# ginevracoal/robustBNNs

Measured on AMD Instinct MI355X. Metric: attack-samples/sec (test_pts x posterior_samples x PGD_iters), higher is better.
Workload: dtype f32 (full-width operands as three f16 pieces: 6 exact f16 MFMA product terms per fp32 product, f32 accumulate)

## Files before the change

### robustbnns_amd/csrc/rbnn_triple.hip

```cpp
#include "rbnn_common.hpp"
#include <algorithm>
#include <cstdlib>

namespace {

__device__ __forceinline__ void split3(float v, _Float16& p0, _Float16& p1, _Float16& p2) {
    p0 = (_Float16)v;
    float r = v - (float)p0;
    p1 = (_Float16)r;
    r -= (float)p1;
    p2 = (_Float16)r;
}

#ifndef RBNN_X3_PAIR_NOP
#define RBNN_X3_PAIR_NOP 0
#endif
#if RBNN_X3_PAIR_NOP
#define RBNN_X3_PAIR_PAD "\n\ts_nop 1"
#else
#define RBNN_X3_PAIR_PAD ""
#endif
#define RBNN_X3_PAIR_BODY \
    "v_bfe_i32 %[me], %[mw], %[b0], 1\n\t" \
    "v_bfe_i32 %[mo], %[mw], %[b1], 1\n\t" \
// ... 27 lines not shown
    "v_fma_mix_f32 %[re], %[ge], %[me], -%[d0] op_sel_hi:[0,0,1]\n\t" \
    "v_fma_mix_f32 %[ro], %[go], %[mo], -%[d0] op_sel:[0,0,1] op_sel_hi:[0,0,1]\n\t" \
    "v_cvt_pk_f16_f32 %[d1], %[re], %[ro]\n\t" \
    "v_fma_mixlo_f16 %[d2], -%[d1], %[one], %[re] op_sel_hi:[1,0,0]\n\t" \
    "v_fma_mixhi_f16 %[d2], -%[d1], %[one], %[ro] op_sel:[1,0,0] op_sel_hi:[1,0,0]" RBNN_X3_PAIR_PAD
#define RBNN_X3_PAIRM_OPS \
    : [d0] "=&v"(d0), [d1] "=&v"(d1), [d2] "=&v"(d2), [re] "=&v"(re), [ro] "=&v"(ro) \
    : [ge] "v"(ge), [go] "v"(go), [me] "v"(me), [mo] "v"(mo), [one] "v"(one)
    if constexpr (FIRST) asm volatile("s_nop 7\n\t" RBNN_X3_PAIRM_BODY RBNN_X3_PAIRM_OPS);
    else asm volatile(RBNN_X3_PAIRM_BODY RBNN_X3_PAIRM_OPS);
}


__global__ void triple_rows_kernel(const float* __restrict__ src, long long rows, int cols, int ld_src, float scale,
                                   const rbnn_dev_scale* __restrict__ ds, uint4* __restrict__ dst, int groups, int grouped) {
    const long long i = (long long)blockIdx.x * blockDim.x + threadIdx.x;
    if (i >= rows * groups) return;
    if (ds) scale = ds->scale;
    const long long r = i / groups;
    const int g = (int)(i % groups);
    const float* const p = src + r * ld_src + 8 * g;
    union { f16x8 v; uint4 u; } o[3];
#pragma unroll
    for (int j = 0; j < 8; ++j) {
        const float v = (8 * g + j < cols) ? p[j] * scale : 0.f;
        _Float16 a, b, c;
        split3(v, a, b, c);
        o[0].v[j] = a; o[1].v[j] = b; o[2].v[j] = c;
    }
    if (grouped) {
        uint4* const out = dst + (((r >> 4) * (groups >> 2) + (g >> 2)) * 192 + (r & 15) * 4 + (g & 3));
        out[0] = o[0].u; out[64] = o[1].u; out[128] = o[2].u;
        return;
    }
    uint4* const out = dst + (r * (groups >> 2) + (g >> 2)) * 12 + (g & 3);
    out[0] = o[0].u; out[4] = o[1].u; out[8] = o[2].u;
}

struct FwdX3Args {
    const char* X;  int ldx;  int N;
    const char* W;  long long w_sample_bytes;  int ldw;  int KT;
    const float* b;  const float* W2;  const float* b2;  int C;  int H;
    const int* sidx;  int S;  int NT;  float out_scale;
    float* P;  uint32_t* mask;  float* dact;  int out_kind;
    const rbnn_dev_scale* x_ds;
    long long x_sample_bytes;  char* hid;  float hid_scale;  const rbnn_dev_scale* hid_ds;
    unsigned x_group_bytes, x_stage_bytes;
};

template <int ACT, int WH, int HTW, int WN, int NTW, bool LAYER2, bool XF32 = false>
__global__ void __launch_bounds__(64 * WH * WN, WH * WN / 4) fc_forward_x3_kernel(const FwdX3Args a) {
    constexpr int BH = WH * HTW * 16, BN = WN * NTW * 16;
    constexpr int PLANEB = (BH + BN) * 64;
    constexpr int TILEB = 3 * PLANEB;
    constexpr bool BITMASK = (ACT == RBNN_ACT_RELU || ACT == RBNN_ACT_LEAKY);
    constexpr int NW = WH * WN;
    constexpr int WPP = BH / 16 / NW, XPP = BN / 16 / NW;
    static_assert((BH / 16) % NW == 0 && (BN / 16) % NW == 0, "whole pieces per wave");
    static_assert(HTW % 2 == 0 && HTW <= 8, "a wave's h range is whole 32-bit mask words, at most 4");
    static_assert(WH * BN * 64 <= 2 * TILEB, "the Z^T reduction scratch aliases the tile buffers");
    extern __shared__ __attribute__((aligned(16))) float lds[];
    char* const ldsb = (char*)lds;
    float* const zred = lds;

    int id;
    if (!item_of_block(blockIdx.x, a.NT * a.S, id)) return;
    constexpr int SB = 4;
    int ntile, s;
    {
        const int full = a.S / SB, per = SB * a.NT;
        if (id < full * per) { ntile = (id % per) / SB; s = (id / per) * SB + id % SB; }
        else { const int rem = id - full * per, cnt = a.S - full * SB; ntile = rem / cnt; s = full * SB + rem % cnt; }
    }
    const int tid = threadIdx.x, lane = tid & 63, li = lane & 15, lg = lane >> 4;
    const int wave = __builtin_amdgcn_readfirstlane(tid >> 6);
    const int wave_h = wave % WH, wave_n = wave / WH;
    const int sw = a.sidx ? a.sidx[s] : s;
    const float out_scale = a.x_ds ? a.out_scale * a.x_ds->inv_scale : a.out_scale;
    const float hid_scale = (!LAYER2 && a.hid_ds) ? a.hid_ds->scale : a.hid_scale;
    const char* const Ws = a.W + (long long)sw * a.w_sample_bytes;
    const char* const Xs = a.X + (long long)s * a.x_sample_bytes;
    const int n0 = ntile * BN;
    const int HW = a.H >> 5;
    const int prow = lane >> 2;
    const unsigned src_off = (unsigned)(prow * 64 + ((lane & 3) ^ swz(prow)) * 16);
    const int foff = li * 64 + ((lg ^ swz(li)) * 16);
    auto sw8 = [](int r) { return ((r >> 1) & 1) | (((r >> 2) & 1) << 2); };
    const unsigned src_off_f = (unsigned)((lane >> 3) * 128 + (((lane & 7) ^ sw8(lane >> 3)) * 16));
    const int foff_f0 = li * 128 + (((2 * lg) ^ sw8(li)) * 16), foff_f1 = li * 128 + (((2 * lg + 1) ^ sw8(li)) * 16);

    f32x4 zacc[NTW];
#pragma unroll
    for (int nt = 0; nt < NTW; ++nt) zacc[nt] = (f32x4){0.f, 0.f, 0.f, 0.f};
    if (NW == 8 && wave >= 4) __builtin_amdgcn_s_setprio(1);

    unsigned xrow[XPP], wrow[WPP];
#pragma unroll
    for (int i = 0; i < XPP; ++i) xrow[i] = (unsigned)min((n0 >> 4) + wave + NW * i, ((a.N + 15) >> 4) - 1) * a.x_group_bytes + (XF32 ? src_off_f : src_off);
#pragma unroll
    for (int i = 0; i < WPP; ++i) wrow[i] = (unsigned)(wave + NW * i) * (unsigned)a.KT * 3072u + src_off;

    constexpr int PPS = WPP + XPP;
    const int G = (a.H / BH) * a.KT;
    auto piece = [&](int c, int kt, int buf, int j) {
        char* const T = ldsb + buf * TILEB;
        const char* src;
        char* dst;
        if (j < WPP) {
            src = Ws + (long long)c * BH * a.ldw * 6 + (wrow[j < WPP ? j : 0] + (unsigned)kt * 3072u);
            dst = T + (wave + NW * j) * 3072;
        } else {
            src = Xs + (xrow[j >= WPP ? j - WPP : 0] + (unsigned)kt * a.x_stage_bytes);
            dst = T + (BH / 16 + wave + NW * (j - WPP)) * 3072;
        }
        const auto gsrc = (const __attribute__((address_space(1))) void*)src;
        const auto ldst = (__attribute__((address_space(3))) void*)(uintptr_t)(uint32_t)(uintptr_t)dst;
        __builtin_amdgcn_global_load_lds(gsrc, ldst, 16, 0, 0);
        __builtin_amdgcn_global_load_lds(gsrc, ldst, 16, 1024, 0);
        if (!(XF32 && j >= WPP)) __builtin_amdgcn_global_load_lds(gsrc, ldst, 16, 2048, 0);
    };
#pragma unroll
    for (int i = 0; i < PPS; ++i) piece(0, 0, 0, i);
    ring_wait_barrier<0>();

    f32x4 acc[HTW][NTW];
#pragma unroll
    for (int ht = 0; ht < HTW; ++ht)
#pragma unroll
        for (int nt = 0; nt < NTW; ++nt) acc[ht][nt] = (f32x4){0.f, 0.f, 0.f, 0.f};

    int kt = 0, ch = 0;
    for (int g = 0; g < G; ++g) {
        const int buf = g & 1;
        const bool wrap = kt + 1 == a.KT, last = g + 1 == G;
        const int ktn = last ? kt : (wrap ? 0 : kt + 1), chn = (wrap && !last) ? ch + 1 : ch;
        const char* const Wt = ldsb + buf * TILEB + (wave_h * HTW) * 3072 + foff;
        const char* const Xt = ldsb + buf * TILEB + (BH / 16 + wave_n * NTW) * 3072 + foff;
        f16x8 b0[NTW], b1[NTW], b2[NTW], a0, a1, a2, a0n, a1n, a2n;
        if (!(RBNN_ABL & 1)) {
#pragma unroll
            for (int i = 0; i < PPS; ++i) piece(chn, ktn, buf ^ 1, i);
        }
        if constexpr (XF32) {
            const char* const Xf = ldsb + buf * TILEB + (BH / 16 + wave_n * NTW) * 3072;
            f32x4 x0[NTW], x1[NTW];
#pragma unroll
            for (int nt = 0; nt < NTW; ++nt) {
                x0[nt] = *(const f32x4*)(Xf + nt * 3072 + foff_f0);
                x1[nt] = *(const f32x4*)(Xf + nt * 3072 + foff_f1);
            }
#pragma unroll
            for (int nt = 0; nt < NTW; ++nt) {
                union { f16x8 v; unsigned w[4]; } q0, q1, q2;
                split3_plain_pair(x0[nt][0], x0[nt][1], 1.f, q0.w[0], q1.w[0], q2.w[0]);
                split3_plain_pair(x0[nt][2], x0[nt][3], 1.f, q0.w[1], q1.w[1], q2.w[1]);
                split3_plain_pair(x1[nt][0], x1[nt][1], 1.f, q0.w[2], q1.w[2], q2.w[2]);
                split3_plain_pair(x1[nt][2], x1[nt][3], 1.f, q0.w[3], q1.w[3], q2.w[3]);
                b0[nt] = q0.v; b1[nt] = q1.v; b2[nt] = q2.v;
            }
        } else {
#pragma unroll
            for (int nt = 0; nt < NTW; ++nt) {
                b0[nt] = *(const f16x8*)(Xt + nt * 3072);
                b1[nt] = *(const f16x8*)(Xt + nt * 3072 + 1024);
                b2[nt] = *(const f16x8*)(Xt + nt * 3072 + 2048);
            }
        }
        a0 = *(const f16x8*)(Wt);
        a1 = *(const f16x8*)(Wt + 1024);
        a2 = *(const f16x8*)(Wt + 2048);
        a0n = a0; a1n = a1; a2n = a2;
#pragma unroll
        for (int ht = 0; ht < HTW; ++ht) {
#pragma unroll
            for (int k = 0; k < 6; ++k) {
                const f16x8 av = (k == 1) ? a2 : ((k == 2 || k == 3) ? a1 : a0);
#pragma unroll
                for (int nt = 0; nt < NTW; ++nt) {
                    const f16x8 bv = (k == 0) ? b2[nt] : ((k == 2 || k == 4) ? b1[nt] : b0[nt]);
                    acc[ht][nt] = MFMA_H(av, bv, acc[ht][nt]);
                }
                if (k == 0 && ht + 1 < HTW) {
                    a0n = *(const f16x8*)(Wt + (ht + 1) * 3072);
                    a1n = *(const f16x8*)(Wt + (ht + 1) * 3072 + 1024);
                    a2n = *(const f16x8*)(Wt + (ht + 1) * 3072 + 2048);
                }
            }
            a0 = a0n; a1 = a1n; a2 = a2n;
        }
        {
            __builtin_amdgcn_sched_group_barrier(0x100, 3 * NTW + 3, 0);
#pragma unroll
            for (int ht = 0; ht < HTW; ++ht) {
                __builtin_amdgcn_sched_group_barrier(0x008, 3 * NTW, 0);
                if (ht + 1 < HTW) __builtin_amdgcn_sched_group_barrier(0x100, 3, 0);
                __builtin_amdgcn_sched_group_barrier(0x008, 3 * NTW, 0);
            }
        }
        if (!(RBNN_ABL & 2)) ring_wait_barrier<0>();
        const int hc0 = ch * BH;
        kt = wrap ? 0 : kt + 1;
        ch = wrap ? ch + 1 : ch;
        if (!wrap) continue;

        if (RBNN_ABL & 8) {
            float t = 0.f;
#pragma unroll
            for (int ht = 0; ht < HTW; ++ht)
#pragma unroll
                for (int nt = 0; nt < NTW; ++nt) { t += acc[ht][nt][0] + acc[ht][nt][1] + acc[ht][nt][2] + acc[ht][nt][3]; acc[ht][nt] = (f32x4){0.f, 0.f, 0.f, 0.f}; }
            if (t == 12345.678f) a.P[tid] = t;
            continue;
        }
        const int hw0 = hc0 + (wave_h * HTW) * 16;
        unsigned mine[NTW];
#pragma unroll
        for (int nt = 0; nt < NTW; ++nt) mine[nt] = 0u;
#pragma unroll
        for (int ht = 0; ht < HTW; ++ht) {
            const int hrow = hw0 + ht * 16 + 4 * lg;
            const f32x4 bias = *(const f32x4*)(a.b + (long long)sw * a.H + hrow);
            f32x4 w2f = (f32x4){0.f, 0.f, 0.f, 0.f};
            if (LAYER2 && li < a.C) w2f = *(const f32x4*)(a.W2 + ((long long)sw * a.C + li) * a.H + hrow);
#pragma unroll
            for (int nt = 0; nt < NTW; ++nt) {
                const int n = n0 + (wave_n * NTW + nt) * 16 + li;
                f32x4 v = acc[ht][nt] * out_scale + bias, hv;
                acc[ht][nt] = (f32x4){0.f, 0.f, 0.f, 0.f};
                unsigned bits = 0;
#pragma unroll
                for (int r = 0; r < 4; ++r) {
                    bits |= (v[r] > 0.f ? 1u : 0u) << r;
                    hv[r] = act_fwd<ACT>(v[r]);
                }
                if (BITMASK) {
                    unsigned part = bits << (16 * (ht & 1) + 4 * lg);
                    part |= __shfl_xor(part, 16);
                    part |= __shfl_xor(part, 32);
                    if (lg == (ht >> 1)) mine[nt] |= part;
                }
                if (!BITMASK && a.dact && n < a.N) {
                    f32x4 dv;
#pragma unroll
                    for (int r = 0; r < 4; ++r) dv[r] = act_grad_from_value<ACT>(hv[r]);
                    *(f32x4*)(a.dact + ((long long)s * a.N + n) * a.H + hrow) = dv;
                }
                if (LAYER2) {
#pragma unroll
                    for (int r = 0; r < 4; ++r) zacc[nt] = MFMA16(w2f[r], hv[r], zacc[nt]);
                } else {
#ifdef RBNN_X3_L1_ABL_NOSTORE
                    if (n < a.N && hv[0] == 1.2345e-30f) {
#else
                    if (n < a.N) {
#endif
                        const long long blk = ((long long)s * HW + (hrow >> 5)) * ((a.N + 15) >> 4) + (n >> 4);
#ifdef RBNN_X3_L1_ABL_SMALL
                        char* const row = a.hid + ((blk * 2048) & 0xFFC00) + (n & 15) * 128 + ((hrow >> 4) & 1) * 64 + lg * 16;
#else
                        char* const row = a.hid + blk * 2048 + (n & 15) * 128 + ((hrow >> 4) & 1) * 64 + lg * 16;
#endif
                        *(f32x4*)row = hv * hid_scale;
                    }
                }
            }
        }
        if (BITMASK && a.mask) {
#pragma unroll
            for (int nt = 0; nt < NTW; ++nt) {
                const int n = n0 + (wave_n * NTW + nt) * 16 + li;
                if (lg < HTW / 2 && n < a.N) a.mask[((long long)s * HW + (hw0 >> 5) + lg) * mask_ld(a.N) + n] = mine[nt];
            }
        }
    }
    if (RBNN_ABL & 2) ring_wait_barrier<0>();

    if (!LAYER2) return;
#pragma unroll
    for (int nt = 0; nt < NTW; ++nt)
        *(f32x4*)(zred + (wave_h * BN + (wave_n * NTW + nt) * 16 + li) * 16 + 4 * lg) = zacc[nt];
    __syncthreads();
    if (tid < BN) {
        const int n = n0 + tid;
        float z[16];
#pragma unroll
        for (int q = 0; q < 4; ++q) {
            f32x4 sum = *(const f32x4*)(zred + tid * 16 + 4 * q);
#pragma unroll
            for (int w = 1; w < WH; ++w) sum += *(const f32x4*)(zred + (w * BN + tid) * 16 + 4 * q);
#pragma unroll
            for (int r = 0; r < 4; ++r) z[4 * q + r] = sum[r];
        }
        float m = -INFINITY;
#pragma unroll
        for (int c = 0; c < 16; ++c) {
            if (c < a.C) { z[c] += a.b2[(long long)sw * a.C + c]; m = fmaxf(m, z[c]); }
            else z[c] = 0.f;
        }
        if (a.out_kind == RBNN_OUT_PROBS) {
            float den = 0.f;
#pragma unroll
            for (int c = 0; c < 16; ++c) if (c < a.C) { z[c] = expf(z[c] - m); den += z[c]; }
#pragma unroll
            for (int c = 0; c < 16; ++c) if (c < a.C) z[c] = z[c] / den;
        }
        if (n < a.N) {
            float* const dst = a.P + ((long long)s * a.N + n) * RBNN_CPAD;
#pragma unroll
            for (int q = 0; q < 4; ++q) *(f32x4*)(dst + 4 * q) = (f32x4){z[4 * q], z[4 * q + 1], z[4 * q + 2], z[4 * q + 3]};
        }
    }
}

template <int ACT, int WH, int HTW, int WN, int NTW, bool LAYER2, bool XF32>
int launch_forward_x3_cfg(FwdX3Args a, hipStream_t st) {
    constexpr int BH = WH * HTW * 16, BN = WN * NTW * 16;
    constexpr int LDSB = 2 * 3 * (BH + BN) * 64;
    static_assert(LDSB <= 160 * 1024, "LDS");
    a.NT = (a.N + BN - 1) / BN;
    auto kern = fc_forward_x3_kernel<ACT, WH, HTW, WN, NTW, LAYER2, XF32>;
    static unsigned long long attr_done = 0;
    if (!ensure_dynamic_lds((const void*)kern, LDSB, attr_done)) return RBNN_ERR_LAUNCH;
    const int grid = grid_for_items((long long)a.NT * a.S);
    hipLaunchKernelGGL(kern, dim3(grid), dim3(64 * WH * WN), LDSB, st, a);
    return launch_status();
}

template <int ACT, bool LAYER2, bool XF32>
int launch_forward_x3_act(const FwdX3Args& a, hipStream_t st) {
    if (a.H % 256 == 0) return launch_forward_x3_cfg<ACT, 4, 4, 2, 4, LAYER2, XF32>(a, st);
    if (a.H % 128 == 0) return launch_forward_x3_cfg<ACT, 2, 4, 2, 4, LAYER2, XF32>(a, st);
    return RBNN_ERR_UNSUPPORTED;
}

template <bool LAYER2, bool XF32 = false>
int launch_forward_x3(int act, const FwdX3Args& a, hipStream_t st) {
    switch (act) {
#ifndef RBNN_FAST_BUILD
        case RBNN_ACT_RELU:  return launch_forward_x3_act<RBNN_ACT_RELU, LAYER2, XF32>(a, st);
#endif
        case RBNN_ACT_LEAKY: return launch_forward_x3_act<RBNN_ACT_LEAKY, LAYER2, XF32>(a, st);
#ifndef RBNN_FAST_BUILD
        case RBNN_ACT_SIGM:  return launch_forward_x3_act<RBNN_ACT_SIGM, LAYER2, XF32>(a, st);
        case RBNN_ACT_TANH:  return launch_forward_x3_act<RBNN_ACT_TANH, LAYER2, XF32>(a, st);
#endif
    }
    return RBNN_ERR_UNSUPPORTED;
}

__global__ void triple_cols_kernel(const float* __restrict__ W, long long n_mats, int rows, int cols, int ld_src, float scale,
                                   uint4* __restrict__ dst, int ld_dst) {
    const long long i = (long long)blockIdx.x * blockDim.x + threadIdx.x;
    const int HB = rows / 32;
    if (i >= n_mats * HB * 4 * ld_dst) return;
    const int d = (int)(i % ld_dst);
    const int lg = (int)((i / ld_dst) % 4);
    const long long mh = i / (4LL * ld_dst);
// ... 21 lines not shown
    const int t = (int)((i >> 7) % (H / 16));
    const long long m = (i >> 7) / (H / 16);
    _Float16 w[3][10];
#pragma unroll
    for (int c = 0; c < 10; ++c) {
        const float v = (c < C) ? W2[(m * C + c) * H + 16 * t + li] * scale : 0.f;
        split3(v, w[0][c], w[1][c], w[2][c]);
    }
    union { f16x8 v; uint4 u; } o;
    const _Float16 z = (_Float16)0.f;
    if (lg < 3) {
        const int piece = (k == 0) ? (lg == 2 ? 1 : 0) : (lg == 0 ? 1 : (lg == 1 ? 0 : 2));
#pragma unroll
        for (int j = 0; j < 8; ++j) o.v[j] = piece == 0 ? w[0][j] : (piece == 1 ? w[1][j] : w[2][j]);
    } else if (k == 0) {
        o.v[0] = w[0][8]; o.v[1] = w[0][9]; o.v[2] = w[0][8]; o.v[3] = w[0][9];
        o.v[4] = w[0][8]; o.v[5] = w[0][9]; o.v[6] = w[1][8]; o.v[7] = w[1][9];
    } else {
        o.v[0] = w[2][8]; o.v[1] = w[2][9]; o.v[2] = w[1][8]; o.v[3] = w[1][9];
        o.v[4] = z; o.v[5] = z; o.v[6] = z; o.v[7] = z;
    }
    dst[i] = o.u;
}

__host__ __device__ __forceinline__ int dz_swz3(long long n) { return (int)((0 - (n >> 2)) & 3); }

__global__ void __launch_bounds__(256) triple_dz_kernel(const float* __restrict__ dZ, int S, int N, long long N_pad, int C,
                                                        uint4* __restrict__ dst, float* __restrict__ gscale) {
    __shared__ float red[16][17];
    const int p = threadIdx.x & 15, q = threadIdx.x >> 4;
    const long long n = (long long)blockIdx.x * 16 + p;
    float m = 0.f;
    if (n < N)
        for (int s = q; s < S; s += 16) {
            const float* const src = dZ + ((long long)s * N + n) * RBNN_CPAD;
#pragma unroll
            for (int k = 0; k < 3; ++k) {
                const f32x4 v = *(const f32x4*)(src + 4 * k);
#pragma unroll
                for (int r = 0; r < 4; ++r) if (4 * k + r < C) m = fmaxf(m, fabsf(v[r]));
            }
        }
    red[q][p] = m;
    __syncthreads();
    m = 0.f;
#pragma unroll
    for (int i = 0; i < 16; ++i) m = fmaxf(m, red[i][p]);
    int e = 0;
    if (m > 0.f && m < INFINITY) e = min(13 - ilogbf(m), 120);
    if (q == 0) gscale[n] = ldexpf(1.f, -e);
    const int sw = dz_swz3(n);
    for (int s = q; s < S; s += 16) {
        _Float16 d[3][10];
        float v[12];
        if (n < N) {
            const float* const src = dZ + ((long long)s * N + n) * RBNN_CPAD;
#pragma unroll
            for (int k = 0; k < 3; ++k) {
                const f32x4 t = *(const f32x4*)(src + 4 * k);
#pragma unroll
                for (int r = 0; r < 4; ++r) v[4 * k + r] = t[r];
            }
        }
#pragma unroll
        for (int c = 0; c < 10; ++c) {
            const float x = (n < N && c < C) ? ldexpf(v[c], e) : 0.f;
            split3(x, d[0][c], d[1][c], d[2][c]);
        }
        uint4* const o = dst + ((long long)s * N_pad + n) * 4;
#pragma unroll
        for (int ch = 0; ch < 3; ++ch) {
            union { f16x8 v; uint4 u; } w;
#pragma unroll
            for (int j = 0; j < 8; ++j) w.v[j] = d[ch][j];
            o[ch ^ sw] = w.u;
        }
        union { f16x8 v; uint4 u; } t;
        t.v[0] = d[0][8]; t.v[1] = d[0][9]; t.v[2] = d[1][8]; t.v[3] = d[1][9];
        t.v[4] = d[2][8]; t.v[5] = d[2][9]; t.v[6] = d[0][8]; t.v[7] = d[0][9];
        o[3 ^ sw] = t.u;
    }
}

template <int MODE>
__device__ __forceinline__ void tail_dz(const float* __restrict__ prow, const float (&gmean)[16], int y, int C, float inv_S, float (&out)[16]) {
    float p[16], g[16];
#pragma unroll
    for (int q = 0; q < 4; ++q) {
        const f32x4 v = *(const f32x4*)(prow + 4 * q);
#pragma unroll
        for (int r = 0; r < 4; ++r) p[4 * q + r] = v[r];
    }
    if (MODE == RBNN_LOSS_PER_SAMPLE) {
        ce_softmax_grad<16>(p, C, y, inv_S, g);
    } else {
#pragma unroll
        for (int c = 0; c < 16; ++c) g[c] = gmean[c];
    }
    if (MODE == RBNN_LOSS_MEAN_LOGIT) {
#pragma unroll
        for (int c = 0; c < 16; ++c) out[c] = g[c];
    } else {
        softmax_backward<16>(g, p, C, out);
    }
}

template <int MODE>
__global__ void __launch_bounds__(256) step_tail_x3_kernel(const float* __restrict__ P, const int* __restrict__ labels, int S, float inv_S, int N,
                                                           long long N_pad, int C, float* __restrict__ Psum_out, int ldo,
                                                           uint4* __restrict__ dst, float* __restrict__ gscale) {
    __shared__ float red[16][17];
    __shared__ float psum[16][16];
    const int p = threadIdx.x & 15, q = threadIdx.x >> 4;
    const long long n = (long long)blockIdx.x * 16 + p;
    if (MODE != RBNN_LOSS_PER_SAMPLE) {
        if (q < 4) {
            f32x4 sum = (f32x4){0.f, 0.f, 0.f, 0.f};
            if (n < N)
                for (int s = 0; s < S; ++s) sum += *(const f32x4*)(P + ((long long)s * N + n) * RBNN_CPAD + 4 * q);
#pragma unroll
            for (int r = 0; r < 4; ++r) {
                psum[p][4 * q + r] = sum[r];
                if (Psum_out && n < N && 4 * q + r < C) Psum_out[n * ldo + 4 * q + r] = sum[r];
            }
        }
        __syncthreads();
    }
    const int y = (n < N) ? labels[n] : 0;
    float gmean[16];
    if (MODE != RBNN_LOSS_PER_SAMPLE) {
        float t[16];
#pragma unroll
        for (int c = 0; c < 16; ++c) t[c] = (c < C) ? psum[p][c] * inv_S : 0.f;
        ce_softmax_grad<16>(t, C, y, inv_S, gmean);
    } else {
#pragma unroll
        for (int c = 0; c < 16; ++c) gmean[c] = 0.f;
    }
    float m = 0.f;
    if (n < N)
        for (int s = q; s < S; s += 16) {
            float dz[16];
            tail_dz<MODE>(P + ((long long)s * N + n) * RBNN_CPAD, gmean, y, C, inv_S, dz);
#pragma unroll
            for (int c = 0; c < 12; ++c) if (c < C) m = fmaxf(m, fabsf(dz[c]));
        }
    red[q][p] = m;
    __syncthreads();
    m = 0.f;
#pragma unroll
    for (int i = 0; i < 16; ++i) m = fmaxf(m, red[i][p]);
    int e = 0;
    if (m > 0.f && m < INFINITY) e = min(13 - ilogbf(m), 120);
    if (q == 0) gscale[n] = ldexpf(1.f, -e);
    const int sw = dz_swz3(n);
    for (int s = q; s < S; s += 16) {
        _Float16 d[3][10];
        float dz[16];
#pragma unroll
        for (int c = 0; c < 16; ++c) dz[c] = 0.f;
        if (n < N) tail_dz<MODE>(P + ((long long)s * N + n) * RBNN_CPAD, gmean, y, C, inv_S, dz);
#pragma unroll
        for (int c = 0; c < 10; ++c) {
            const float x = (n < N && c < C) ? ldexpf(dz[c], e) : 0.f;
            split3(x, d[0][c], d[1][c], d[2][c]);
        }
        uint4* const o = dst + ((long long)s * N_pad + n) * 4;
#pragma unroll
        for (int ch = 0; ch < 3; ++ch) {
            union { f16x8 v; uint4 u; } w;
#pragma unroll
            for (int j = 0; j < 8; ++j) w.v[j] = d[ch][j];
            o[ch ^ sw] = w.u;
        }
        union { f16x8 v; uint4 u; } t;
        t.v[0] = d[0][8]; t.v[1] = d[0][9]; t.v[2] = d[1][8]; t.v[3] = d[1][9];
        t.v[4] = d[2][8]; t.v[5] = d[2][9]; t.v[6] = d[0][8]; t.v[7] = d[0][9];
        o[3 ^ sw] = t.u;
    }
}

__global__ void __launch_bounds__(256) attack_step_x3_kernel(float* __restrict__ X, const float* __restrict__ X0, int ldx, const float* __restrict__ G,
                                                             int K, long long slab_stride, int ldg, const float* __restrict__ alpha, float alpha_scalar,
                                                             float eps, int project, long long N, int D, const rbnn_dev_scale* __restrict__ ds,
                                                             uint4* __restrict__ dst, int groups) {
    const long long i = (long long)blockIdx.x * blockDim.x + threadIdx.x;
    if (i >= N * groups) return;
    const long long n = i / groups;
    const int gq = (int)(i % groups), d0 = 8 * gq;
    const float scale = ds->scale;
    float xn[8];
#pragma unroll
    for (int j = 0; j < 8; ++j) xn[j] = 0.f;
    if (d0 < D) {
        const float step = alpha ? alpha[n] : alpha_scalar;
#pragma unroll
        for (int h = 0; h < 2; ++h) {
            const int d = d0 + 4 * h;
            if (d < D) {
                f32x4 g = *(const f32x4*)(G + n * ldg + d);
                for (int k = 1; k < K; ++k) g += *(const f32x4*)(G + k * slab_stride + n * ldg + d);
                const f32x4 x = *(const f32x4*)(X + n * ldx + d);
                f32x4 x0 = x, out;
                if (project) x0 = *(const f32x4*)(X0 + n * ldx + d);
#pragma unroll
                for (int r = 0; r < 4; ++r) {
                    const float sgn = (g[r] > 0.f) ? 1.f : ((g[r] < 0.f) ? -1.f : 0.f);
                    float pert = x[r] + step * sgn;
                    if (project) pert = x0[r] + fminf(fmaxf(pert - x0[r], -eps), eps);
                    out[r] = fminf(fmaxf(pert, 0.f), 1.f);
                    xn[4 * h + r] = out[r];
                }
                *(f32x4*)(X + n * ldx + d) = out;
            }
        }
    }
    union { f16x8 v; uint4 u; } o[3];
#pragma unroll
    for (int j = 0; j < 8; ++j) {
        const float v = (d0 + j < D) ? xn[j] * scale : 0.f;
        _Float16 a, b, c;
        split3(v, a, b, c);
        o[0].v[j] = a; o[1].v[j] = b; o[2].v[j] = c;
    }
    uint4* const out = dst + (((n >> 4) * (groups >> 2) + (gq >> 2)) * 192 + (n & 15) * 4 + (gq & 3));
    out[0] = o[0].u; out[64] = o[1].u; out[128] = o[2].u;
}

#define GEN_Q3 (-17)

struct GradX3Args {
    const char* dzg;  long long n_pad;  const float* gscale;  const uint32_t* mask;
    const char* W1c;  int ldc;
    const char* W2g;
    int H;  int HW;  const int* sidx;  int S;  int chunk;  int nchunks;
    int N;  int NT;  int ND;  int Dt;
    float* out;  int ldo;  float out_scale;
    const uint32_t* omask;  int OHW;
    const float* amem;
    const float* dact;  const float* odact;
};
enum { X3_FC = 0, X3_FC2_STEP1 = 1, X3_FC2_STEP2 = 2 };

template <int ACT, int TD, int MODE>
__global__ void __launch_bounds__(256, 2) fc_grad_x3_kernel(const GradX3Args a) {
    constexpr int NW = 4;
    constexpr bool GEN = MODE != X3_FC2_STEP2;
    constexpr bool BITMASK = (ACT == RBNN_ACT_RELU || ACT == RBNN_ACT_LEAKY);
    constexpr bool STREAM = !GEN || !BITMASK;
    constexpr int NTW = 16 / NW, BM = 256, LD = TD * 16;
    constexpr int W1B = 12 * LD * 16;
    constexpr int NPIECE = W1B / 1024, PPW = (NPIECE + NW - 1) / NW;
    constexpr int BUFB = W1B + 4096 + 1024;
    constexpr int DZB = BM * 64;
    static_assert(W1B % 1024 == 0, "whole DMA pieces");
    extern __shared__ __attribute__((aligned(16))) float lds[];
    char* const ldsb = (char*)lds;
    char* const dzl = ldsb + 2 * BUFB;

    int id;
    if (!item_of_block(blockIdx.x, a.NT * a.ND * a.nchunks, id)) return;
    int ntile, dg, ch;
    grad_item(id, a.NT, a.ND, STREAM, ntile, dg, ch);
    const int tid = threadIdx.x, lane = tid & 63, li = lane & 15, lg = lane >> 4;
    const int wave = __builtin_amdgcn_readfirstlane(tid >> 6);
    const int nb = ntile * BM + wave * (NTW * 16);
    const int dc0 = dg * LD;
    const int Dp = a.Dt * 16;
    const int ntd = min(TD, a.Dt - dg * TD);
    const int s_begin = ch * a.chunk, s_end = min(a.S, s_begin + a.chunk);
    const int HS = a.H / 32, nst = (s_end - s_begin) * HS;

    unsigned goff[PPW];
#pragma unroll
    for (int i = 0; i < PPW; ++i) {
        const int f = (wave + NW * i) * 1024 + lane * 16, seg = f / (LD * 16), d = (f % (LD * 16)) >> 4;
        goff[i] = (unsigned)(seg * a.ldc + min(dc0 + d, a.ldc - 1)) * 16u;
    }
    const unsigned loff = (unsigned)lane * 16u;

    f32x4 acc[NTW][TD];
#pragma unroll
    for (int nt = 0; nt < NTW; ++nt)
#pragma unroll
        for (int dt = 0; dt < TD; ++dt) acc[nt][dt] = (f32x4){0.f, 0.f, 0.f, 0.f};

    auto dz_issue = [&](int s) {
        const char* const src = a.dzg + ((long long)s * a.n_pad + nb) * 64;
#pragma unroll
        for (int j = 0; j < NTW; ++j) glds16((const float*)(src + j * 1024 + loff), (float*)(dzl + wave * (NTW * 1024) + j * 1024));
    };
    constexpr int NDMA = GEN ? (BITMASK ? PPW + 2 : PPW + 1) : PPW;
    struct StageSrc { const char* W; const char* G; const char* M; char* B; };
    auto stage_src = [&](int st, int buf) {
        const int si = st / HS, hb = st % HS, s = s_begin + si;
        const int sw = a.sidx ? a.sidx[s] : s;
        StageSrc r;
        r.W = a.W1c + ((long long)sw * HS + hb) * 12 * a.ldc * 16;
        r.G = a.W2g + ((long long)sw * (a.H / 16) + 2 * hb) * 2048 + wave * 1024;
        r.M = (const char*)(a.mask + ((long long)s * a.HW + hb) * a.n_pad + ntile * BM);
        r.B = ldsb + buf * BUFB;
        return r;
    };
    auto issue_piece = [&](const StageSrc& q, int i) {
        if (i < PPW) {
            if (wave + NW * i < NPIECE) glds16((const float*)(q.W + goff[i < PPW ? i : 0]), (float*)(q.B + (wave + NW * i) * 1024));
        } else if (i == PPW) {
            glds16((const float*)(q.G + loff), (float*)(q.B + W1B + wave * 1024));
        } else if (BITMASK && i == PPW + 1) {
            if (wave == NW - 1) glds16((const float*)(q.M + loff), (float*)(q.B + W1B + 4096));
        }
    };

    if (GEN) dz_issue(s_begin);
    {
        const StageSrc q = stage_src(0, 0);
#pragma unroll
        for (int i = 0; i < NDMA; ++i) issue_piece(q, i);
    }
    f32x4 am[STREAM ? NTW : 1][2];
    auto load_a = [&](int st) {
        const int s = s_begin + st / HS, h0 = (st % HS) * 32;
        const float* const base = GEN ? a.dact : a.amem;
#pragma unroll
        for (int nt = 0; nt < (STREAM ? NTW : 0); ++nt) {
            const int n = min(nb + nt * 16 + li, a.N - 1);
            const float* const src = base + ((long long)s * a.N + n) * a.H + h0 + 4 * lg;
            am[nt][0] = *(const f32x4*)src;
            am[nt][1] = *(const f32x4*)(src + 16);
        }
    };
    if (STREAM) load_a(0);
    ring_wait_barrier<0>();
    const float c_pos = ldexpf(1.f, GEN_Q3);
    const unsigned cp_bits = __float_as_uint(c_pos);
    const unsigned cn_bits = (ACT == RBNN_ACT_RELU) ? 0u : __float_as_uint(LEAKY_SLOPE * ldexpf(1.f, GEN_Q3));
    const int dzc1 = (lg == 2 ? 0 : lg), dzc2 = (lg == 0 ? 1 : (lg == 1 ? 2 : (lg == 2 ? 0 : 3)));
    const int sz = dz_swz3(li);
    const char* const dzw = dzl + wave * (NTW * 1024) + li * 64;
    f16x8 da0[NTW], da1[NTW], da2[NTW];
    for (int st = 0; st < nst; ++st) {
        const int buf = st & 1, hb = st % HS;
        const bool more = !(RBNN_ABL & 1) && st + 1 < nst;
        const StageSrc q = stage_src(more ? st + 1 : st, buf ^ 1);
        const char* const B = ldsb + buf * BUFB;
        const bool gen_on = GEN && (!(RBNN_ABL & 16) || st == 0);
        if (!GEN) {
#pragma unroll
            for (int nt = 0; nt < (GEN ? 0 : NTW); ++nt) {
                union { f16x8 v; unsigned u[4]; } o0, o1, o2;
#pragma unroll
                for (int t = 0; t < 2; ++t) {
                    split3_plain_pair(am[nt][t][0], am[nt][t][1], 1.f, o0.u[2 * t], o1.u[2 * t], o2.u[2 * t]);
                    split3_plain_pair(am[nt][t][2], am[nt][t][3], 1.f, o0.u[2 * t + 1], o1.u[2 * t + 1], o2.u[2 * t + 1]);
                }
                da0[nt] = o0.v; da1[nt] = o1.v; da2[nt] = o2.v;
            }
        }
        if (more) {
#pragma unroll
            for (int i = 0; i < NDMA; ++i) issue_piece(q, i);
        }
        f32x4 dm[(GEN && STREAM) ? NTW : 1][2];
        if (GEN && STREAM) {
#pragma unroll
            for (int nt = 0; nt < ((GEN && STREAM) ? NTW : 0); ++nt) { dm[nt][0] = am[nt][0] * c_pos; dm[nt][1] = am[nt][1] * c_pos; }
        }
        if (STREAM && st + 1 < nst) load_a(st + 1);

        if (gen_on) {
            const f16x8 w00 = *(const f16x8*)(B + W1B + lane * 16);
            const f16x8 w01 = *(const f16x8*)(B + W1B + 1024 + lane * 16);
            const f16x8 w10 = *(const f16x8*)(B + W1B + 2048 + lane * 16);
            const f16x8 w11 = *(const f16x8*)(B + W1B + 3072 + lane * 16);
            const unsigned* const Mk = (const unsigned*)(B + W1B + 4096) + wave * (NTW * 16) + li;
#pragma unroll
            for (int nt = 0; nt < NTW; ++nt) {
                const f16x8 dz1 = *(const f16x8*)(dzw + nt * 1024 + ((dzc1 ^ sz) * 16));
                const f16x8 dz2 = *(const f16x8*)(dzw + nt * 1024 + ((dzc2 ^ sz) * 16));
                const f32x4 z = (f32x4){0.f, 0.f, 0.f, 0.f};
                const f32x4 g0 = MFMA_H(w01, dz2, MFMA_H(w00, dz1, z)), g1 = MFMA_H(w11, dz2, MFMA_H(w10, dz1, z));
                union { f16x8 v; unsigned u[4]; } o0, o1, o2;
                if constexpr (BITMASK) {
                    const unsigned mw = Mk[nt * 16] >> (4 * lg);
                    split3_pair<0, true>(g0[0], g0[1], mw, cp_bits, cn_bits, 1.f, o0.u[0], o1.u[0], o2.u[0]);
                    split3_pair<2, false>(g0[2], g0[3], mw, cp_bits, cn_bits, 1.f, o0.u[1], o1.u[1], o2.u[1]);
                    split3_pair<16, true>(g1[0], g1[1], mw, cp_bits, cn_bits, 1.f, o0.u[2], o1.u[2], o2.u[2]);
                    split3_pair<18, false>(g1[2], g1[3], mw, cp_bits, cn_bits, 1.f, o0.u[3], o1.u[3], o2.u[3]);
                } else {
                    constexpr int q = (GEN && STREAM) ? 1 : 0;
                    split3_pair_m<true>(g0[0], g0[1], dm[q * nt][0][0], dm[q * nt][0][1], 1.f, o0.u[0], o1.u[0], o2.u[0]);
                    split3_pair_m<false>(g0[2], g0[3], dm[q * nt][0][2], dm[q * nt][0][3], 1.f, o0.u[1], o1.u[1], o2.u[1]);
                    split3_pair_m<true>(g1[0], g1[1], dm[q * nt][1][0], dm[q * nt][1][1], 1.f, o0.u[2], o1.u[2], o2.u[2]);
                    split3_pair_m<false>(g1[2], g1[3], dm[q * nt][1][2], dm[q * nt][1][3], 1.f, o0.u[3], o1.u[3], o2.u[3]);
                }
                da0[nt] = o0.v; da1[nt] = o1.v; da2[nt] = o2.v;
            }
        }
        if (GEN && !(RBNN_ABL & 1) && hb == HS - 1 && st + 1 < nst) {
            asm volatile("" ::: "memory");
            __builtin_amdgcn_s_waitcnt(0xC07F);
            asm volatile("" ::: "memory");
            dz_issue(s_begin + st / HS + 1);
        }
        const char* const Bw = B + (lg * 3 * LD + li) * 16;
        f16x8 bb[2][3];
        bb[0][0] = *(const f16x8*)(Bw); bb[0][1] = *(const f16x8*)(Bw + LD * 16); bb[0][2] = *(const f16x8*)(Bw + 2 * LD * 16);
#pragma unroll
        for (int dt = 0; dt < TD; ++dt) {
            if (dt < ntd) {
                f16x8 (&bc)[3] = bb[dt & 1];
                if (dt + 1 < TD) {
                    f16x8 (&bn)[3] = bb[(dt + 1) & 1];
                    bn[0] = *(const f16x8*)(Bw + (dt + 1) * 256);
                    bn[1] = *(const f16x8*)(Bw + LD * 16 + (dt + 1) * 256);
                    bn[2] = *(const f16x8*)(Bw + 2 * LD * 16 + (dt + 1) * 256);
                }
#pragma unroll
                for (int nt = 0; nt < NTW; ++nt) acc[nt][dt] = MFMA_H(da0[nt], bc[2], acc[nt][dt]);
#pragma unroll
                for (int nt = 0; nt < NTW; ++nt) acc[nt][dt] = MFMA_H(da2[nt], bc[0], acc[nt][dt]);
#pragma unroll
                for (int nt = 0; nt < NTW; ++nt) acc[nt][dt] = MFMA_H(da1[nt], bc[1], acc[nt][dt]);
#pragma unroll
                for (int nt = 0; nt < NTW; ++nt) acc[nt][dt] = MFMA_H(da1[nt], bc[0], acc[nt][dt]);
#pragma unroll
                for (int nt = 0; nt < NTW; ++nt) acc[nt][dt] = MFMA_H(da0[nt], bc[1], acc[nt][dt]);
#pragma unroll
                for (int nt = 0; nt < NTW; ++nt) acc[nt][dt] = MFMA_H(da0[nt], bc[0], acc[nt][dt]);
            }
        }
        if (!(RBNN_ABL & 2)) ring_wait_barrier<0>();
    }
    if (RBNN_ABL & 2) ring_wait_barrier<0>();

    if (RBNN_ABL & 8) {
        float t = 0.f;
#pragma unroll
        for (int nt = 0; nt < NTW; ++nt)
#pragma unroll
            for (int dt = 0; dt < TD; ++dt) t += acc[nt][dt][0] + acc[nt][dt][1] + acc[nt][dt][2] + acc[nt][dt][3];
        if (t == 12345.678f) a.out[tid] = t;
        return;
    }
    constexpr int LDW = LD + 4, C4 = LD / 4, E4 = 16 * C4;
    static_assert(NW * 16 * LDW * 4 <= 2 * BUFB + DZB, "the waves' transposition tiles fit the loop buffers");
    float* const tw = (float*)ldsb + wave * (16 * LDW);
#pragma unroll
    for (int nt = 0; nt < NTW; ++nt) {
#pragma unroll
        for (int r = 0; r < 4; ++r) {
            const int n = nb + nt * 16 + 4 * lg + r;
            const float gs = (MODE == X3_FC2_STEP1) ? a.out_scale : (n < a.N ? a.gscale[n] : 0.f) * a.out_scale;
#pragma unroll
            for (int dt = 0; dt < TD; ++dt) tw[(4 * lg + r) * LDW + dt * 16 + li] = acc[nt][dt][r] * gs;
        }
#pragma unroll
        for (int i = 0; i < (E4 + 63) / 64; ++i) {
            const int e4 = i * 64 + lane, row = e4 / C4, c4 = e4 - row * C4;
            const int n = nb + nt * 16 + row, d = dc0 + 4 * c4;
            if (e4 < E4 && n < a.N && d < Dp) {
                f32x4 v = *(const f32x4*)(tw + row * LDW + 4 * c4);
                if (MODE == X3_FC2_STEP1) {
                    if (BITMASK) {
                        const unsigned w = a.omask[((long long)ch * a.OHW + (d >> 5)) * a.n_pad + n] >> (d & 31);
#pragma unroll
                        for (int k = 0; k < 4; ++k) v[k] = ((w >> k) & 1u) ? v[k] : (ACT == RBNN_ACT_RELU ? 0.f : v[k] * LEAKY_SLOPE);
                    } else {
                        v *= *(const f32x4*)(a.odact + ((long long)ch * a.N + n) * a.ldo + d);
                    }
                }
                *(f32x4*)(a.out + ((long long)ch * a.N + n) * a.ldo + d) = v;
            }
        }
    }
}

template <int ACT, int TD, int MODE>
int launch_grad_x3_cfg(GradX3Args a, hipStream_t st) {
    constexpr int LDSB = 2 * (12 * TD * 16 * 16 + 5120) + 256 * 64;
    static_assert(2 * LDSB <= 160 * 1024, "two blocks per CU");
    a.NT = (a.N + 255) / 256;
    a.ND = (a.Dt + TD - 1) / TD;
    auto kern = fc_grad_x3_kernel<ACT, TD, MODE>;
    static unsigned long long attr_done = 0;
    if (!ensure_dynamic_lds((const void*)kern, LDSB, attr_done)) return RBNN_ERR_LAUNCH;
    const int grid = grid_for_items((long long)a.NT * a.ND * a.nchunks);
    hipLaunchKernelGGL(kern, dim3(grid), dim3(256), LDSB, st, a);
    return launch_status();
}

inline bool x3_grad_td9() {
    static const bool on = [] { const char* e = getenv("RBNN_X3_GRAD_TD9"); return !e || e[0] != '0'; }();
    return on;
}

template <int ACT, int TD, int MODE>
bool x3_grad_two_blocks() {
    static int ok[64] = {0};
    int dev = 0;
    if (hipGetDevice(&dev) != hipSuccess || dev < 0 || dev >= 64) return false;
    if (!ok[dev]) {
        constexpr int LDSB = 2 * (12 * TD * 16 * 16 + 5120) + 256 * 64;
        auto kern = fc_grad_x3_kernel<ACT, TD, MODE>;
        static unsigned long long attr_done = 0;
        int nb = 0;
        const bool fine = ensure_dynamic_lds((const void*)kern, LDSB, attr_done) &&
                          hipOccupancyMaxActiveBlocksPerMultiprocessor(&nb, kern, 256, LDSB) == hipSuccess && nb >= 2;
        ok[dev] = fine ? 1 : 2;
    }
    return ok[dev] == 1;
}

template <int ACT, int MODE>
int launch_grad_x3(const GradX3Args& a, hipStream_t st) {
    if constexpr (MODE == X3_FC && (ACT == RBNN_ACT_RELU || ACT == RBNN_ACT_LEAKY)) {
// ... 208 lines not shown
```

Baseline: 136.7 million.

## Skip MFMA work on out-of-range N tiles and prefetch tail-kernel sample rows

The forward and backward triple-split GEMM loops are templated into three variants: full tiles, partially valid tiles and fully empty tiles. Partial variants skip loads, splits and MFMAs for 16-column subtiles past N, avoiding wasted tensor-core work on the ragged last tile. The tail reduction kernels gain a register ring and a one-step prefetch of per-sample probability rows to hide global-load latency. This adds code-size and register pressure from the duplicated loop bodies. In main_part the loop bound NTW-1 looks suspicious, since it may skip a valid last subtile.

```diff
diff --git a/robustbnns_amd/csrc/rbnn_triple.hip b/robustbnns_amd/csrc/rbnn_triple.hip
--- a/robustbnns_amd/csrc/rbnn_triple.hip
+++ b/robustbnns_amd/csrc/rbnn_triple.hip
@@ -133,6 +133,7 @@
     const char* const Xs = a.X + (long long)s * a.x_sample_bytes;
     const int n0 = ntile * BN;
     const int HW = a.H >> 5;
+    const int nvf = min(max((a.N - n0 - wave_n * (NTW * 16) + 15) >> 4, 0), NTW);
     const int prow = lane >> 2;
     const unsigned src_off = (unsigned)(prow * 64 + ((lane & 3) ^ swz(prow)) * 16);
     const int foff = li * 64 + ((lg ^ swz(li)) * 16);
@@ -180,79 +181,93 @@
 #pragma unroll
         for (int nt = 0; nt < NTW; ++nt) acc[ht][nt] = (f32x4){0.f, 0.f, 0.f, 0.f};
 
+    auto stage_mma = [&](auto full, const int buf) {
+        constexpr bool FULL = decltype(full)::value;
+        const char* const Wt = ldsb + buf * TILEB + (wave_h * HTW) * 3072 + foff;
+        const char* const Xt = ldsb + buf * TILEB + (BH / 16 + wave_n * NTW) * 3072 + foff;
+        f16x8 b0[NTW], b1[NTW], b2[NTW], a0, a1, a2, a0n, a1n, a2n;
+            if constexpr (XF32) {
+                const char* const Xf = ldsb + buf * TILEB + (BH / 16 + wave_n * NTW) * 3072;
+                f32x4 x0[NTW], x1[NTW];
+    #pragma unroll
+                for (int nt = 0; nt < NTW; ++nt) {
+                    if (FULL || nt < nvf) {
+                        x0[nt] = *(const f32x4*)(Xf + nt * 3072 + foff_f0);
+                        x1[nt] = *(const f32x4*)(Xf + nt * 3072 + foff_f1);
+                    }
+                }
+    #pragma unroll
+                for (int nt = 0; nt < NTW; ++nt) {
+                    if (FULL || nt < nvf) {
+                        union { f16x8 v; unsigned w[4]; } q0, q1, q2;
+                        split3_plain_pair(x0[nt][0], x0[nt][1], 1.f, q0.w[0], q1.w[0], q2.w[0]);
+                        split3_plain_pair(x0[nt][2], x0[nt][3], 1.f, q0.w[1], q1.w[1], q2.w[1]);
+                        split3_plain_pair(x1[nt][0], x1[nt][1], 1.f, q0.w[2], q1.w[2], q2.w[2]);
+                        split3_plain_pair(x1[nt][2], x1[nt][3], 1.f, q0.w[3], q1.w[3], q2.w[3]);
+                        b0[nt] = q0.v; b1[nt] = q1.v; b2[nt] = q2.v;
+                    }
+                }
+            } else {
+    #pragma unroll
+                for (int nt = 0; nt < NTW; ++nt) {
+                    if (FULL || nt < nvf) {
+                        b0[nt] = *(const f16x8*)(Xt + nt * 3072);
+                        b1[nt] = *(const f16x8*)(Xt + nt * 3072 + 1024);
+                        b2[nt] = *(const f16x8*)(Xt + nt * 3072 + 2048);
+                    }
+                }
+            }
+            a0 = *(const f16x8*)(Wt);
+            a1 = *(const f16x8*)(Wt + 1024);
+            a2 = *(const f16x8*)(Wt + 2048);
+            a0n = a0; a1n = a1; a2n = a2;
+    #pragma unroll
+            for (int ht = 0; ht < HTW; ++ht) {
+    #pragma unroll
+                for (int k = 0; k < 6; ++k) {
+                    const f16x8 av = (k == 1) ? a2 : ((k == 2 || k == 3) ? a1 : a0);
+    #pragma unroll
+                    for (int nt = 0; nt < NTW; ++nt) {
+                        if (FULL || nt < nvf) {
+                            const f16x8 bv = (k == 0) ? b2[nt] : ((k == 2 || k == 4) ? b1[nt] : b0[nt]);
+                            acc[ht][nt] = MFMA_H(av, bv, acc[ht][nt]);
+                        }
+                    }
+                    if (k == 0 && ht + 1 < HTW) {
+                        a0n = *(const f16x8*)(Wt + (ht + 1) * 3072);
+                        a1n = *(const f16x8*)(Wt + (ht + 1) * 3072 + 1024);
+                        a2n = *(const f16x8*)(Wt + (ht + 1) * 3072 + 2048);
+                    }
+                }
+                a0 = a0n; a1 = a1n; a2 = a2n;
+            }
+            if constexpr (FULL) {
+                __builtin_amdgcn_sched_group_barrier(0x100, 3 * NTW + 3, 0);
+    #pragma unroll
+                for (int ht = 0; ht < HTW; ++ht) {
+                    __builtin_amdgcn_sched_group_barrier(0x008, 3 * NTW, 0);
+                    if (ht + 1 < HTW) __builtin_amdgcn_sched_group_barrier(0x100, 3, 0);
+                    __builtin_amdgcn_sched_group_barrier(0x008, 3 * NTW, 0);
+                }
+            }
+    };
     int kt = 0, ch = 0;
-    for (int g = 0; g < G; ++g) {
+    auto stage = [&](auto kind, const int g) {
+        constexpr int KIND = decltype(kind)::value;
         const int buf = g & 1;
         const bool wrap = kt + 1 == a.KT, last = g + 1 == G;
         const int ktn = last ? kt : (wrap ? 0 : kt + 1), chn = (wrap && !last) ? ch + 1 : ch;
-        const char* const Wt = ldsb + buf * TILEB + (wave_h * HTW) * 3072 + foff;
-        const char* const Xt = ldsb + buf * TILEB + (BH / 16 + wave_n * NTW) * 3072 + foff;
-        f16x8 b0[NTW], b1[NTW], b2[NTW], a0, a1, a2, a0n, a1n, a2n;
         if (!(RBNN_ABL & 1)) {
 #pragma unroll
             for (int i = 0; i < PPS; ++i) piece(chn, ktn, buf ^ 1, i);
         }
-        if constexpr (XF32) {
-            const char* const Xf = ldsb + buf * TILEB + (BH / 16 + wave_n * NTW) * 3072;
-            f32x4 x0[NTW], x1[NTW];
-#pragma unroll
-            for (int nt = 0; nt < NTW; ++nt) {
-                x0[nt] = *(const f32x4*)(Xf + nt * 3072 + foff_f0);
-                x1[nt] = *(const f32x4*)(Xf + nt * 3072 + foff_f1);
-            }
-#pragma unroll
-            for (int nt = 0; nt < NTW; ++nt) {
-                union { f16x8 v; unsigned w[4]; } q0, q1, q2;
-                split3_plain_pair(x0[nt][0], x0[nt][1], 1.f, q0.w[0], q1.w[0], q2.w[0]);
-                split3_plain_pair(x0[nt][2], x0[nt][3], 1.f, q0.w[1], q1.w[1], q2.w[1]);
-                split3_plain_pair(x1[nt][0], x1[nt][1], 1.f, q0.w[2], q1.w[2], q2.w[2]);
-                split3_plain_pair(x1[nt][2], x1[nt][3], 1.f, q0.w[3], q1.w[3], q2.w[3]);
-                b0[nt] = q0.v; b1[nt] = q1.v; b2[nt] = q2.v;
-            }
-        } else {
-#pragma unroll
-            for (int nt = 0; nt < NTW; ++nt) {
-                b0[nt] = *(const f16x8*)(Xt + nt * 3072);
-                b1[nt] = *(const f16x8*)(Xt + nt * 3072 + 1024);
-                b2[nt] = *(const f16x8*)(Xt + nt * 3072 + 2048);
-            }
-        }
-        a0 = *(const f16x8*)(Wt);
-        a1 = *(const f16x8*)(Wt + 1024);
-        a2 = *(const f16x8*)(Wt + 2048);
-        a0n = a0; a1n = a1; a2n = a2;
-#pragma unroll
-        for (int ht = 0; ht < HTW; ++ht) {
-#pragma unroll
-            for (int k = 0; k < 6; ++k) {
-                const f16x8 av = (k == 1) ? a2 : ((k == 2 || k == 3) ? a1 : a0);
-#pragma unroll
-                for (int nt = 0; nt < NTW; ++nt) {
-                    const f16x8 bv = (k == 0) ? b2[nt] : ((k == 2 || k == 4) ? b1[nt] : b0[nt]);
-                    acc[ht][nt] = MFMA_H(av, bv, acc[ht][nt]);
-                }
-                if (k == 0 && ht + 1 < HTW) {
-                    a0n = *(const f16x8*)(Wt + (ht + 1) * 3072);
-                    a1n = *(const f16x8*)(Wt + (ht + 1) * 3072 + 1024);
-                    a2n = *(const f16x8*)(Wt + (ht + 1) * 3072 + 2048);
-                }
-            }
-            a0 = a0n; a1 = a1n; a2 = a2n;
-        }
-        {
-            __builtin_amdgcn_sched_group_barrier(0x100, 3 * NTW + 3, 0);
-#pragma unroll
-            for (int ht = 0; ht < HTW; ++ht) {
-                __builtin_amdgcn_sched_group_barrier(0x008, 3 * NTW, 0);
-                if (ht + 1 < HTW) __builtin_amdgcn_sched_group_barrier(0x100, 3, 0);
-                __builtin_amdgcn_sched_group_barrier(0x008, 3 * NTW, 0);
-            }
-        }
+        if constexpr (KIND == 2) stage_mma(std::true_type{}, buf);
+        else if constexpr (KIND == 1) stage_mma(std::false_type{}, buf);
         if (!(RBNN_ABL & 2)) ring_wait_barrier<0>();
         const int hc0 = ch * BH;
         kt = wrap ? 0 : kt + 1;
         ch = wrap ? ch + 1 : ch;
-        if (!wrap) continue;
+        if (!wrap) return;
 
         if (RBNN_ABL & 8) {
             float t = 0.f;
@@ -261,7 +276,7 @@
 #pragma unroll
                 for (int nt = 0; nt < NTW; ++nt) { t += acc[ht][nt][0] + acc[ht][nt][1] + acc[ht][nt][2] + acc[ht][nt][3]; acc[ht][nt] = (f32x4){0.f, 0.f, 0.f, 0.f}; }
             if (t == 12345.678f) a.P[tid] = t;
-            continue;
+            return;
         }
         const int hw0 = hc0 + (wave_h * HTW) * 16;
         unsigned mine[NTW];
@@ -323,7 +338,10 @@
                 if (lg < HTW / 2 && n < a.N) a.mask[((long long)s * HW + (hw0 >> 5) + lg) * mask_ld(a.N) + n] = mine[nt];
             }
         }
-    }
+    };
+    if (nvf == NTW) { for (int g = 0; g < G; ++g) stage(std::integral_constant<int, 2>{}, g); }
+    else if (nvf > 0) { for (int g = 0; g < G; ++g) stage(std::integral_constant<int, 1>{}, g); }
+    else { for (int g = 0; g < G; ++g) stage(std::integral_constant<int, 0>{}, g); }
     if (RBNN_ABL & 2) ring_wait_barrier<0>();
 
     if (!LAYER2) return;
@@ -511,14 +529,21 @@
     }
 }
 
+struct TailRow { f32x4 v[4]; };
+__device__ __forceinline__ TailRow tail_row(const float* __restrict__ prow) {
+    TailRow t;
+#pragma unroll
+    for (int q = 0; q < 4; ++q) t.v[q] = *(const f32x4*)(prow + 4 * q);
+    return t;
+}
+
 template <int MODE>
-__device__ __forceinline__ void tail_dz(const float* __restrict__ prow, const float (&gmean)[16], int y, int C, float inv_S, float (&out)[16]) {
+__device__ __forceinline__ void tail_dz(const TailRow& row, const float (&gmean)[16], int y, int C, float inv_S, float (&out)[16]) {
     float p[16], g[16];
 #pragma unroll
     for (int q = 0; q < 4; ++q) {
-        const f32x4 v = *(const f32x4*)(prow + 4 * q);
-#pragma unroll
-        for (int r = 0; r < 4; ++r) p[4 * q + r] = v[r];
+#pragma unroll
+        for (int r = 0; r < 4; ++r) p[4 * q + r] = row.v[q][r];
     }
     if (MODE == RBNN_LOSS_PER_SAMPLE) {
         ce_softmax_grad<16>(p, C, y, inv_S, g);
@@ -544,9 +569,25 @@
     const long long n = (long long)blockIdx.x * 16 + p;
     if (MODE != RBNN_LOSS_PER_SAMPLE) {
         if (q < 4) {
+            constexpr int RING = 16;
             f32x4 sum = (f32x4){0.f, 0.f, 0.f, 0.f};
-            if (n < N)
-                for (int s = 0; s < S; ++s) sum += *(const f32x4*)(P + ((long long)s * N + n) * RBNN_CPAD + 4 * q);
+            if (n < N) {
+                const float* const src = P + n * RBNN_CPAD + 4 * q;
+                const long long ss = (long long)N * RBNN_CPAD;
+                f32x4 ring[RING];
+#pragma unroll
+                for (int j = 0; j < RING; ++j)
+                    if (j < S) ring[j] = *(const f32x4*)(src + j * ss);
+                for (int s0 = 0; s0 < S; s0 += RING) {
+#pragma unroll
+                    for (int j = 0; j < RING; ++j) {
+                        if (s0 + j < S) {
+                            sum += ring[j];
+                            if (s0 + j + RING < S) ring[j] = *(const f32x4*)(src + (s0 + j + RING) * ss);
+                        }
+                    }
+                }
+            }
 #pragma unroll
             for (int r = 0; r < 4; ++r) {
                 psum[p][4 * q + r] = sum[r];
@@ -566,14 +607,20 @@
 #pragma unroll
         for (int c = 0; c < 16; ++c) gmean[c] = 0.f;
     }
+    const float* const prow = P + n * RBNN_CPAD;
+    const long long pss = (long long)N * RBNN_CPAD;
     float m = 0.f;
-    if (n < N)
+    if (n < N && q < S) {
+        TailRow nxt = tail_row(prow + q * pss);
         for (int s = q; s < S; s += 16) {
+            const TailRow cur = nxt;
+            if (s + 16 < S) nxt = tail_row(prow + (s + 16) * pss);
             float dz[16];
-            tail_dz<MODE>(P + ((long long)s * N + n) * RBNN_CPAD, gmean, y, C, inv_S, dz);
+            tail_dz<MODE>(cur, gmean, y, C, inv_S, dz);
 #pragma unroll
             for (int c = 0; c < 12; ++c) if (c < C) m = fmaxf(m, fabsf(dz[c]));
         }
+    }
     red[q][p] = m;
     __syncthreads();
     m = 0.f;
@@ -583,12 +630,18 @@
     if (m > 0.f && m < INFINITY) e = min(13 - ilogbf(m), 120);
     if (q == 0) gscale[n] = ldexpf(1.f, -e);
     const int sw = dz_swz3(n);
+    TailRow nxt;
+    if (n < N && q < S) nxt = tail_row(prow + q * pss);
     for (int s = q; s < S; s += 16) {
         _Float16 d[3][10];
         float dz[16];
 #pragma unroll
         for (int c = 0; c < 16; ++c) dz[c] = 0.f;
-        if (n < N) tail_dz<MODE>(P + ((long long)s * N + n) * RBNN_CPAD, gmean, y, C, inv_S, dz);
+        if (n < N) {
+            const TailRow cur = nxt;
+            if (s + 16 < S) nxt = tail_row(prow + (s + 16) * pss);
+            tail_dz<MODE>(cur, gmean, y, C, inv_S, dz);
+        }
 #pragma unroll
         for (int c = 0; c < 10; ++c) {
             const float x = (n < N && c < C) ? ldexpf(dz[c], e) : 0.f;
@@ -697,6 +750,7 @@
     const int dc0 = dg * LD;
     const int Dp = a.Dt * 16;
     const int ntd = min(TD, a.Dt - dg * TD);
+    const int ntv = min(max((a.N - nb + 15) >> 4, 0), NTW);
     const int s_begin = ch * a.chunk, s_end = min(a.S, s_begin + a.chunk);
     const int HS = a.H / 32, nst = (s_end - s_begin) * HS;
 
@@ -768,15 +822,11 @@
     const int sz = dz_swz3(li);
     const char* const dzw = dzl + wave * (NTW * 1024) + li * 64;
     f16x8 da0[NTW], da1[NTW], da2[NTW];
-    for (int st = 0; st < nst; ++st) {
-        const int buf = st & 1, hb = st % HS;
-        const bool more = !(RBNN_ABL & 1) && st + 1 < nst;
-        const StageSrc q = stage_src(more ? st + 1 : st, buf ^ 1);
-        const char* const B = ldsb + buf * BUFB;
-        const bool gen_on = GEN && (!(RBNN_ABL & 16) || st == 0);
-        if (!GEN) {
-#pragma unroll
-            for (int nt = 0; nt < (GEN ? 0 : NTW); ++nt) {
+    auto split_a = [&](auto full) {
+        constexpr bool FULL = decltype(full)::value;
+#pragma unroll
+        for (int nt = 0; nt < (GEN ? 0 : NTW); ++nt) {
+            if (FULL || nt < ntv) {
                 union { f16x8 v; unsigned u[4]; } o0, o1, o2;
 #pragma unroll
                 for (int t = 0; t < 2; ++t) {
@@ -786,25 +836,17 @@
                 da0[nt] = o0.v; da1[nt] = o1.v; da2[nt] = o2.v;
             }
         }
-        if (more) {
-#pragma unroll
-            for (int i = 0; i < NDMA; ++i) issue_piece(q, i);
-        }
-        f32x4 dm[(GEN && STREAM) ? NTW : 1][2];
-        if (GEN && STREAM) {
-#pragma unroll
-            for (int nt = 0; nt < ((GEN && STREAM) ? NTW : 0); ++nt) { dm[nt][0] = am[nt][0] * c_pos; dm[nt][1] = am[nt][1] * c_pos; }
-        }
-        if (STREAM && st + 1 < nst) load_a(st + 1);
-
-        if (gen_on) {
-            const f16x8 w00 = *(const f16x8*)(B + W1B + lane * 16);
-            const f16x8 w01 = *(const f16x8*)(B + W1B + 1024 + lane * 16);
-            const f16x8 w10 = *(const f16x8*)(B + W1B + 2048 + lane * 16);
-            const f16x8 w11 = *(const f16x8*)(B + W1B + 3072 + lane * 16);
-            const unsigned* const Mk = (const unsigned*)(B + W1B + 4096) + wave * (NTW * 16) + li;
-#pragma unroll
-            for (int nt = 0; nt < NTW; ++nt) {
+    };
+    auto generate = [&](auto full, const char* const B, const auto& dm) {
+        constexpr bool FULL = decltype(full)::value;
+        const f16x8 w00 = *(const f16x8*)(B + W1B + lane * 16);
+        const f16x8 w01 = *(const f16x8*)(B + W1B + 1024 + lane * 16);
+        const f16x8 w10 = *(const f16x8*)(B + W1B + 2048 + lane * 16);
+        const f16x8 w11 = *(const f16x8*)(B + W1B + 3072 + lane * 16);
+        const unsigned* const Mk = (const unsigned*)(B + W1B + 4096) + wave * (NTW * 16) + li;
+#pragma unroll
+        for (int nt = 0; nt < NTW; ++nt) {
+            if (FULL || nt < ntv) {
                 const f16x8 dz1 = *(const f16x8*)(dzw + nt * 1024 + ((dzc1 ^ sz) * 16));
                 const f16x8 dz2 = *(const f16x8*)(dzw + nt * 1024 + ((dzc2 ^ sz) * 16));
                 const f32x4 z = (f32x4){0.f, 0.f, 0.f, 0.f};
@@ -826,12 +868,8 @@
                 da0[nt] = o0.v; da1[nt] = o1.v; da2[nt] = o2.v;
             }
         }
-        if (GEN && !(RBNN_ABL & 1) && hb == HS - 1 && st + 1 < nst) {
-            asm volatile("" ::: "memory");
-            __builtin_amdgcn_s_waitcnt(0xC07F);
-            asm volatile("" ::: "memory");
-            dz_issue(s_begin + st / HS + 1);
-        }
+    };
+    auto main_full = [&](const char* const B) {
         const char* const Bw = B + (lg * 3 * LD + li) * 16;
         f16x8 bb[2][3];
         bb[0][0] = *(const f16x8*)(Bw); bb[0][1] = *(const f16x8*)(Bw + LD * 16); bb[0][2] = *(const f16x8*)(Bw + 2 * LD * 16);
@@ -859,8 +897,66 @@
                 for (int nt = 0; nt < NTW; ++nt) acc[nt][dt] = MFMA_H(da0[nt], bc[0], acc[nt][dt]);
             }
         }
+    };
+    auto main_part = [&](const char* const B) {
+        const char* const Bw = B + (lg * 3 * LD + li) * 16;
+#pragma unroll
+        for (int dt = 0; dt < TD; ++dt) {
+            if (dt < ntd) {
+                const f16x8 b0 = *(const f16x8*)(Bw + dt * 256), b1 = *(const f16x8*)(Bw + LD * 16 + dt * 256), b2 = *(const f16x8*)(Bw + 2 * LD * 16 + dt * 256);
+#pragma unroll
+                for (int nt = 0; nt < NTW - 1; ++nt) {
+                    if (nt < ntv) {
+                        f32x4 c = MFMA_H(da0[nt], b2, acc[nt][dt]);
+                        c = MFMA_H(da2[nt], b0, c);
+                        c = MFMA_H(da1[nt], b1, c);
+                        c = MFMA_H(da1[nt], b0, c);
+                        c = MFMA_H(da0[nt], b1, c);
+                        acc[nt][dt] = MFMA_H(da0[nt], b0, c);
+                    }
+                }
+            }
+        }
+    };
+    auto stage = [&](auto kind, const int st) {
+        constexpr int KIND = decltype(kind)::value;
+        const int buf = st & 1, hb = st % HS;
+        const bool more = !(RBNN_ABL & 1) && st + 1 < nst;
+        const StageSrc q = stage_src(more ? st + 1 : st, buf ^ 1);
+        const char* const B = ldsb + buf * BUFB;
+        const bool gen_on = GEN && (!(RBNN_ABL & 16) || st == 0);
+        if (!GEN) {
+            if constexpr (KIND == 2) split_a(std::true_type{});
+            else if constexpr (KIND == 1) split_a(std::false_type{});
+        }
+        if (more) {
+#pragma unroll
+            for (int i = 0; i < NDMA; ++i) issue_piece(q, i);
+        }
+        f32x4 dm[(GEN && STREAM) ? NTW : 1][2];
+        if (GEN && STREAM) {
+#pragma unroll
+            for (int nt = 0; nt < ((GEN && STREAM) ? NTW : 0); ++nt) { dm[nt][0] = am[nt][0] * c_pos; dm[nt][1] = am[nt][1] * c_pos; }
+        }
+        if (STREAM && st + 1 < nst) load_a(st + 1);
+
+        if (gen_on) {
+            if constexpr (KIND == 2) generate(std::true_type{}, B, dm);
+            else if constexpr (KIND == 1) generate(std::false_type{}, B, dm);
+        }
+        if (GEN && !(RBNN_ABL & 1) && hb == HS - 1 && st + 1 < nst) {
+            asm volatile("" ::: "memory");
+            __builtin_amdgcn_s_waitcnt(0xC07F);
+            asm volatile("" ::: "memory");
+            dz_issue(s_begin + st / HS + 1);
+        }
+        if constexpr (KIND == 2) main_full(B);
+        else if constexpr (KIND == 1) main_part(B);
         if (!(RBNN_ABL & 2)) ring_wait_barrier<0>();
-    }
+    };
+    if (ntv == NTW) { for (int st = 0; st < nst; ++st) stage(std::integral_constant<int, 2>{}, st); }
+    else if (ntv > 0) { for (int st = 0; st < nst; ++st) stage(std::integral_constant<int, 1>{}, st); }
+    else { for (int st = 0; st < nst; ++st) stage(std::integral_constant<int, 0>{}, st); }
     if (RBNN_ABL & 2) ring_wait_barrier<0>();
 
     if (RBNN_ABL & 8) {
```

New measurement: 133.6 million. -2.2%, worse.
